# JacobYoung115/VisualSLAM

Hardware: AMD Instinct MI355X
Metric: frames/sec @1080p (Harris + DoG keypoint detection) (higher is better)
Workload: dtype u8

## Files before the change

visualslam_amd/csrc/kernels_aux.hip.h:

```cpp
#pragma once
#include <hip/hip_runtime.h>

#include "kernels_generic.hip.h"
#include "kernels_localize.hip.h"

namespace vslam {

__global__ __launch_bounds__(256) void k_resize_linear2x_slide(const uint8_t* __restrict__ src, size_t sstep, size_t sframe,
                                                                uint8_t* __restrict__ dst, size_t dframe, int dpitch,
                                                                int rows, int cols, int seg) {
    const int k = blockIdx.x * 256 + threadIdx.x;
    if (4 * k >= cols) return;
    const bool whole = 4 * k + 3 < cols;
    const int m0 = blockIdx.y * seg, m1 = min(m0 + seg, rows);
    const uint8_t* s = src + blockIdx.z * sframe;
    uint8_t* d = dst + blockIdx.z * dframe + 8 * k;
    const int xl = max(4 * k - 1, 0), xr = min(4 * k + 4, cols - 1);
    auto hrow = [&](int m, uint32_t (&X)[4], uint32_t (&Y)[4]) {
        const uint8_t* r = s + (size_t)min(max(m, 0), rows - 1) * sstep;
        uint32_t w;
        if (whole)
            __builtin_memcpy(&w, r + 4 * k, 4);
        else
            w = (uint32_t)r[4 * k] | ((uint32_t)r[min(4 * k + 1, cols - 1)] << 8) | ((uint32_t)r[min(4 * k + 2, cols - 1)] << 16) |
// ... 12 lines not shown
            Y[i] = pk_lshr_u16(A[i] + (A[i] << 1), 2);
        }
    };
    auto emit = [&](int dy, const uint32_t (&U)[4], const uint32_t (&V)[4]) {
        uint32_t v[4];
#pragma unroll
        for (int i = 0; i < 4; ++i) v[i] = pk_lshr_u16(U[i] + V[i] + 0x00020002u, 2);
        *reinterpret_cast<uint2*>(d + (size_t)dy * dpitch) = make_uint2(v[0] | (v[1] << 8), v[2] | (v[3] << 8));
    };
    uint32_t Xp[4], Yp[4], Xc[4], Yc[4];
    hrow(m0 - 1, Xp, Yp);
    hrow(m0, Xc, Yc);
    for (int m = m0; m < m1; ++m) {
        uint32_t Xn[4], Yn[4];
        hrow(m + 1, Xn, Yn);
        emit(2 * m, Xp, Yc);
        emit(2 * m + 1, Yc, Xn);
#pragma unroll
        for (int i = 0; i < 4; ++i) Xp[i] = Xc[i], Xc[i] = Xn[i], Yc[i] = Yn[i];
    }
}

__global__ __launch_bounds__(256) void k_resize_nearest_half_v4(const uint8_t* __restrict__ src, size_t sframe, int spitch,
                                                                 uint8_t* __restrict__ dst, size_t dframe, int dpitch,
                                                                 int rows, int drows, int dcols) {
    const int k = blockIdx.x * 256 + threadIdx.x;
    const int y = blockIdx.y;
    if (4 * k >= dcols) return;
    const int sy = min(2 * y, rows - 1);
    const uint2 w = *reinterpret_cast<const uint2*>(src + blockIdx.z * sframe + (size_t)sy * spitch + 8 * k);
    *reinterpret_cast<uint32_t*>(dst + blockIdx.z * dframe + (size_t)y * dpitch + 4 * k) =
        even_bytes(w.x, w.y);
}

constexpr int EXT_SPAN = 768;
constexpr int EXT_PITCH = EXT_SPAN + 16;

template <bool LOC>
__global__ __launch_bounds__(256) void k_extrema_w3(const uint8_t* __restrict__ pyr, size_t pframe, ExtGeom g, int o,
                                                     unsigned long long* __restrict__ bits,
                                                     unsigned long long* __restrict__ lflags, size_t bframe, int li0, int li_step) {
    constexpr int NROW = LOC ? 13 : 10;
    __shared__ __attribute__((aligned(16))) uint8_t srow[NROW * EXT_PITCH + 16];
    __shared__ uint2 queue[LOC ? 768 : 1];
    __shared__ uint8_t qkeep[LOC ? 768 : 1];
    const int li = li0 + (int)blockIdx.y * li_step, f = blockIdx.z;
    const int rows = g.rows[o], cols = g.cols[o], pitch = g.pitch[o];
    const uint32_t P = (uint32_t)rows * (uint32_t)pitch;
    const uint8_t* dog = pyr + f * pframe + g.oct_off[o] + (size_t)VSLAM_NUM_LEVELS * P;
    const int ya = max(3 * li - 1, 0), yb = 3 * li;
    const int yc = min(3 * li + 1, rows - 1);
    const int c0 = blockIdx.x * EXT_SPAN - 16;
    const int wave = __builtin_amdgcn_readfirstlane(threadIdx.x >> 6), lane = threadIdx.x & 63;
    const int cpiece = c0 + 16 * lane;
    const bool piece_ok = lane < EXT_PITCH / 16 && cpiece >= 0 && cpiece < cols;
#pragma unroll
    for (int i = 0; i < (NROW + 3) / 4; ++i) {
        const int rl = wave + 4 * i;
        if (rl < NROW) {
            const int lev = rl < 10 ? (rl >> 1) : rl - 9, y = rl < 10 ? ((rl & 1) ? yb : ya) : yc;
            const uint8_t* rowp = dog + (ptrdiff_t)(int)((uint32_t)lev * P + (uint32_t)y * (uint32_t)pitch + (uint32_t)c0);
            if (piece_ok)
                *reinterpret_cast<uint4*>(srow + rl * EXT_PITCH + 16 * lane) =
                    *reinterpret_cast<const uint4*>(rowp + (uint32_t)(16 * lane));
        }
    }
    if (blockIdx.x == 0 && threadIdx.x < 10)
        srow[threadIdx.x * EXT_PITCH + 15] = dog[(threadIdx.x >> 1) * P + (uint32_t)((threadIdx.x & 1) ? yb : ya) * (uint32_t)pitch];
    __syncthreads();
    const int lc = g.lat_cols[o], wpr = g.wpr[o], lr = g.lat_rows[o];
    const int lj = blockIdx.x * 256 + threadIdx.x;
    bool cand[3] = {false, false, false}, listed[3] = {false, false, false};
    unsigned long long wcand[3], wlist[3];
    const unsigned long long owns = __builtin_amdgcn_ballot_w64(lj < lc);
    const int xa = 3 * (int)threadIdx.x - 1 + 16;
    uint32_t self[5];
    uint32_t up[5], left[5];
    {
        const uint32_t s = xa & 3;
        const uint32_t sel = 0x0c000c00u | s | ((s + 1) << 16);
        uint32_t mn[5], mx[5];
#pragma unroll
        for (int l = 0; l < 5; ++l) {
            uint32_t off = (uint32_t)(xa & ~3) + (uint32_t)(2 * l * EXT_PITCH);
            if (l) asm volatile("" : "+v"(off));
            const uint32_t* q0 = reinterpret_cast<const uint32_t*>(srow + off);
            const uint32_t* q1 = q0 + EXT_PITCH / 4;
            const uint32_t v0 = __builtin_amdgcn_perm(q0[1], q0[0], sel), v1 = __builtin_amdgcn_perm(q1[1], q1[0], sel);
            const uint32_t lo = pk_min_u16(v0, v1), hi = pk_max_u16(v0, v1);
            mn[l] = min(lo & 0xffffu, lo >> 16);
            mx[l] = max(hi & 0xffffu, hi >> 16);
            self[l] = v1 >> 16;
            if (LOC) up[l] = v0 >> 16, left[l] = v1 & 0xffffu;
        }
#pragma unroll
        for (int L = 1; L <= 3; ++L) {
            const uint32_t lo = min(mn[L - 1], min(mn[L], mn[L + 1])), hi = max(mx[L - 1], max(mx[L], mx[L + 1]));
            wcand[L - 1] = (__builtin_amdgcn_ballot_w64(self[L] == lo) | __builtin_amdgcn_ballot_w64(self[L] == hi)) & owns;
            if (LOC) cand[L - 1] = lj < lc && (self[L] == lo || self[L] == hi);
            else wlist[L - 1] = wcand[L - 1] & __builtin_amdgcn_ballot_w64((int)self[L] >= g.min_contrast);
        }
    }
    if (LOC) {
        uint2* wq = queue + wave * 192;
        uint8_t* wk = qkeep + wave * 192;
        const int xj = xa + 1;
        const int xr = xj + ((3 * lj + 1 < cols) ? 1 : 0);
        unsigned int nw = 0;
        bool queued[3];
#pragma unroll
        for (int L = 1; L <= 3; ++L) {
            bool nz = false;
            uint32_t dpack = 0;
            if (cand[L - 1]) {
                const uint8_t* r1 = srow + (2 * L + 1) * EXT_PITCH;
                const uint8_t* r2 = srow + (9 + L) * EXT_PITCH;
                const int d_x = (int)left[L] - (int)r1[xr];
                const int d_y = (int)up[L] - (int)r2[xj];
                const int d_s = (int)self[L - 1] - (int)self[L + 1];
                nz = d_x != 0 && d_y != 0 && d_s != 0;
                listed[L - 1] = !nz && self[L] >= 8u;
                dpack = (uint32_t)(d_x + 256) | ((uint32_t)(d_y + 256) << 10) | ((uint32_t)(d_s + 256) << 20);
            }
            const unsigned long long m = __builtin_amdgcn_ballot_w64(nz);
            if (nz) {
                const unsigned int slot = nw + __builtin_amdgcn_mbcnt_hi((uint32_t)(m >> 32), __builtin_amdgcn_mbcnt_lo((uint32_t)m, 0u));
                wq[slot] = make_uint2(dpack, self[L] | ((uint32_t)((L - 1) * 64 + lane) << 8));
            }
            queued[L - 1] = nz;
            nw += (unsigned int)__builtin_popcountll(m);
        }
        if (nw) {
            __builtin_amdgcn_fence(__ATOMIC_RELEASE, "wavefront");
            __builtin_amdgcn_wave_barrier();
            __builtin_amdgcn_fence(__ATOMIC_ACQUIRE, "wavefront");
            for (unsigned int q = lane; q < nw; q += 64) {
                const uint2 e = wq[q];
                int nv;
                wk[e.y >> 8] = feature_point_localization((int)(e.x & 1023u) - 256, (int)((e.x >> 10) & 1023u) - 256,
                                                          (int)(e.x >> 20) - 256, (int)(e.y & 255u), nv, g.loc_lut);
            }
            __builtin_amdgcn_fence(__ATOMIC_RELEASE, "wavefront");
            __builtin_amdgcn_wave_barrier();
            __builtin_amdgcn_fence(__ATOMIC_ACQUIRE, "wavefront");
#pragma unroll
            for (int L = 0; L < 3; ++L)
                if (queued[L]) listed[L] = wk[L * 64 + lane] != 0;
        }
    }
    const int word = blockIdx.x * 4 + wave;
    if (word < wpr) {
        const size_t w0 = f * bframe + g.bits_off[o] + (size_t)li * wpr + word;
#pragma unroll
        for (int L = 0; L < 3; ++L) {
            const unsigned long long wc = wcand[L], wl = LOC ? __builtin_amdgcn_ballot_w64(listed[L]) : wlist[L];
            if (lane == 0) {
                const size_t w = w0 + (size_t)L * lr * wpr;
                if (bits) bits[w] = wc;
                lflags[w] = wl;
            }
        }
    }
}


template <bool FMA>
__device__ __forceinline__ float mad_f32(float a, float b, float c) {
    if constexpr (FMA) return __builtin_fmaf(a, b, c);
    else return a * b + c;
}

template <bool FMA = false>
__device__ __forceinline__ float fast_atan2_deg(float y, float x) {
    const float scale = (float)(180.0 / 3.14159265358979323846);
    const float p1 = 0.9997878412794807f * scale, p3 = -0.3258083974640975f * scale;
    const float p5 = 0.1555786518463281f * scale, p7 = -0.04432655554792128f * scale;
    const float eps = (float)2.2204460492503131e-16;
    const float ax = fabsf(x), ay = fabsf(y);
    float a;
    if (ax >= ay) {
        const float c = ay / (ax + eps), c2 = c * c;
        a = mad_f32<FMA>(mad_f32<FMA>(mad_f32<FMA>(p7, c2, p5), c2, p3), c2, p1) * c;
    } else {
        const float c = ax / (ay + eps), c2 = c * c;
        a = 90.f - mad_f32<FMA>(mad_f32<FMA>(mad_f32<FMA>(p7, c2, p5), c2, p3), c2, p1) * c;
    }
    if (x < 0) a = 180.f - a;
    if (y < 0) a = 360.f - a;
    return a;
}

template <int BINS>
__device__ __forceinline__ int hist_bin(float deg) {
    const float reductionCoeff = (float)BINS / 360.0f;
    const int index = (int)(deg * reductionCoeff);
    return min(max(index, 0), BINS - 1);
}

__device__ __forceinline__ float gradient_magnitude(float gx, float gy) {
    const float xx = gx * gx, yy = gy * gy;
    return sqrt_rn_small_nr(xx + yy);
}

template <class Geom>
__device__ __forceinline__ const uint8_t* level_plane(const uint8_t* __restrict__ pyr, int f, size_t pframe, const Geom& g, int o, int level) {
    return pyr + f * pframe + g.oct_off[o] + (size_t)level * g.rows[o] * g.pitch[o];
}

template <bool FMA>
__global__ __launch_bounds__(256) void k_level_gradients(const uint8_t* __restrict__ g, int gpitch, int rows, int cols,
                                                          float* __restrict__ gx, float* __restrict__ gy,
                                                          float* __restrict__ mag, float* __restrict__ orient) {
    const int c = blockIdx.x * 256 + threadIdx.x;
    const int r = blockIdx.y;
// ... 12 lines not shown
```

visualslam_amd/csrc/kernels_pyramid.hip.h:

```cpp
#pragma once
#include <hip/hip_runtime.h>

#include "kernels_generic.hip.h"

namespace vslam {

template <int TW_, int TH_, int N0, int N1, int N2, int N3, int N4, int N5>
struct PyrCfg {
    static constexpr int TW = TW_, TH = TH_;
    static constexpr int n(int l) { return l == 0 ? N0 : l == 1 ? N1 : l == 2 ? N2 : l == 3 ? N3 : l == 4 ? N4 : N5; }
    static constexpr int cmax(int a, int b) { return a > b ? a : b; }
    static constexpr int NMAX = cmax(cmax(cmax(N0, N1), cmax(N2, N3)), cmax(N4, N5));
    static constexpr int R = (NMAX / 2 + 15) & ~15;
    static constexpr int RQ = (TH + 2 * R) / 4;
    static constexpr int RW = TW + 2 * R;
    static constexpr int RWP = RW + 4;
    static constexpr int r(int l) { return n(l) / 2; }
    static constexpr int delta(int l) { return (R - r(l)) & 3; }
    static constexpr int A(int l) { return (R - r(l)) & ~3; }
    static constexpr int ncg(int l) { return (TW + 2 * r(l) + delta(l) + 3) / 4; }
    static constexpr int m1(int l) { return ((delta(l) + 3 + n(l) - 1) >> 2) + 1; }
    static constexpr int pmax(int l) { return (7 + delta(l) + 2 * r(l)) / 2; }
    static constexpr int nb(int l) { return pmax(l) / 4 + 1; }
    static constexpr int hpp_l(int l) { return cmax(2 * ncg(l), TW / 2 - 4 + 4 * nb(l)); }
    static constexpr int HPP =
        (cmax(cmax(cmax(hpp_l(0), hpp_l(1)), cmax(hpp_l(2), hpp_l(3))), cmax(hpp_l(4), hpp_l(5))) + 15) & ~15;
    static constexpr int T4M = ((3 + NMAX - 1) >> 2) + 1;
    static constexpr int TPM = NMAX + 1;
    static constexpr int LDS_BYTES = (RQ * RWP + TH * HPP) * 4;
    static constexpr int NT = (TH / 4) * (TW / 8);
    static constexpr int NW = NT / 64;
    static_assert(TW % 16 == 0 && TH % 8 == 0 && NT % 256 == 0 && NT <= 1024,
                  "a multiple of four waves, one per SIMD: 384-thread workgroups (384 x 32 tiles) ran 16 % slower, their six waves sit 2-2-1-1");
    static_assert((N0 & 1) && (N1 & 1) && (N2 & 1) && (N3 & 1) && (N4 & 1) && (N5 & 1), "odd kernels");
};

template <class CFG>
struct PyrTaps {
    uint32_t t4[6][4][CFG::T4M];
    uint32_t tp[6][CFG::TPM];
};

template <class CFG, int L>
__device__ __forceinline__ void pyr_level(const PyrTaps<CFG>* __restrict__ taps, const uint32_t* __restrict__ rp,
                                          uint32_t* __restrict__ hp, uint8_t* __restrict__ out, size_t P, int cols,
                                          int pitch, int rows, int tile_x0, int tile_y0, uint32_t (&prev_e)[4][2],
                                          uint32_t (&prev_o)[4][2], uint8_t* __restrict__ next_base, int nrows,
                                          int ncols, int npitch, const uint32_t (&row_off)[4]) {
    constexpr int n = CFG::n(L), dl = CFG::delta(L), A = CFG::A(L);
    constexpr int NCG = CFG::ncg(L), M = CFG::m1(L), NB = CFG::nb(L);
    constexpr int RWP = CFG::RWP, HPP = CFG::HPP, TH = CFG::TH;
    const int tid = threadIdx.x;
    uint32_t z1;
    asm volatile("s_mov_b32 %0, 0" : "=s"(z1));
    const uint32_t* __restrict__ t4 = &taps->t4[L][0][0] + z1;
    const uint4* __restrict__ rp4 = reinterpret_cast<const uint4*>(rp);

    constexpr int NT = CFG::NT;
    constexpr int N1 = NCG * (TH / 4), FULL1 = N1 / NT * NT;
    for (int k = 0; k < (N1 + NT - 1) / NT; ++k) {
        int it = tid + NT * k;
        if (k == N1 / NT) {
            it = FULL1 + (tid + NT - 64 * (L % CFG::NW)) % NT;
            if (it >= N1) break;
        }
        const int cg = it % NCG, rq = it / NCG;
        uint32_t acc[4][4];
#pragma unroll
        for (int j = 0; j < 4; ++j)
#pragma unroll
            for (int c = 0; c < 4; ++c) acc[j][c] = 0;
        const uint4* col = rp4 + (rq + A / 4) * (RWP / 4) + cg + A / 4;
#pragma unroll
        for (int m = 0; m < M; ++m) {
            const uint4 v = col[m * (RWP / 4)];
#pragma unroll
            for (int j = 0; j < 4; ++j) {
                const int s = dl + j, o = s & 3, mm = m - (s >> 2);
                if (mm >= 0 && mm <= ((o + n - 1) >> 2)) {
                    const uint32_t t = t4[o * CFG::T4M + mm];
                    acc[j][0] = udot4(v.x, t, acc[j][0]);
                    acc[j][1] = udot4(v.y, t, acc[j][1]);
                    acc[j][2] = udot4(v.z, t, acc[j][2]);
                    acc[j][3] = udot4(v.w, t, acc[j][3]);
                }
            }
        }
#pragma unroll
        for (int j = 0; j < 4; ++j) {
            uint2 w;
            w.x = __builtin_amdgcn_perm(acc[j][1], acc[j][0], 0x05040100);
            w.y = __builtin_amdgcn_perm(acc[j][3], acc[j][2], 0x05040100);
            *reinterpret_cast<uint2*>(hp + (4 * rq + j) * HPP + 2 * cg) = w;
        }
    }
    __syncthreads();

    uint32_t z2;
    asm volatile("s_mov_b32 %0, 0" : "=s"(z2));
    const uint32_t* __restrict__ tp = &taps->tp[L][0] + z2;
    const int xg = tid % (CFG::TW / 8), rg = tid / (CFG::TW / 8);
    uint32_t acc[4][8];
#pragma unroll
    for (int jr = 0; jr < 4; ++jr)
#pragma unroll
        for (int j = 0; j < 8; ++j) acc[jr][j] = 32768u;
#pragma unroll
    for (int b = 0; b < NB; ++b) {
        uint32_t zb = 0;
        if (CFG::TPM > 40 && (b & 1) == 0) asm volatile("s_mov_b32 %0, 0" : "=s"(zb));
        const uint32_t* __restrict__ tpb = CFG::TPM > 40 ? tp + zb : tp;
#pragma unroll
        for (int jr = 0; jr < 4; ++jr) {
            const uint4 v = *reinterpret_cast<const uint4*>(hp + (4 * rg + jr) * HPP + 4 * xg + 4 * b);
            asm volatile("" ::"v"(v.x), "v"(v.y), "v"(v.z), "v"(v.w));
            const uint32_t vv[4] = {v.x, v.y, v.z, v.w};
#pragma unroll
            for (int pp = 0; pp < 4; ++pp) {
#pragma unroll
                for (int j = 0; j < 8; ++j) {
                    const int e = 2 * (4 * b + pp) - j - dl + 1;
                    if (e >= 0 && e <= n) acc[jr][j] = udot2(vv[pp], tpb[e], acc[jr][j]);
                }
            }
        }
    }
    __syncthreads();

    const int x = tile_x0 + 8 * xg;
#pragma unroll
    for (int jr = 0; jr < 4; ++jr) {
        const int y = tile_y0 + 4 * rg + jr;
        uint32_t g[2], d[2];
#pragma unroll
        for (int hw = 0; hw < 2; ++hw)
            level_pack4(acc[jr][4 * hw], acc[jr][4 * hw + 1], acc[jr][4 * hw + 2], acc[jr][4 * hw + 3], L, g[hw], d[hw], prev_e[jr][hw],
                        prev_o[jr][hw]);
        if (y < rows && x < cols) {
            const uint32_t off = row_off[jr];
            uint8_t* gp = out + (size_t)L * P;
            *reinterpret_cast<uint2*>(gp + off) = make_uint2(g[0], g[1]);
            if (L > 0) {
                uint8_t* dp = out + (size_t)(VSLAM_NUM_LEVELS + L - 1) * P;
                *reinterpret_cast<uint2*>(dp + off) = make_uint2(d[0], d[1]);
            }
            if (L == 3 && next_base && (jr & 1) == 0 && (y >> 1) < nrows && (x >> 1) < ncols)
                *reinterpret_cast<uint32_t*>(next_base + ((uint32_t)(y >> 1) * (uint32_t)npitch + (uint32_t)(x >> 1))) = even_bytes(g[0], g[1]);
        }
    }
}

template <class CFG>
__global__ __launch_bounds__(CFG::NT) void k_pyr_octave(const uint8_t* __restrict__ base, size_t bframe,
                                                     uint8_t* __restrict__ oct_out, size_t pframe, int rows, int cols,
                                                     int pitch, const PyrTaps<CFG>* __restrict__ taps,
                                                     uint8_t* __restrict__ next_base, size_t nframe, int nrows, int ncols,
                                                     int npitch) {
    extern __shared__ __attribute__((aligned(16))) uint32_t smem[];
    uint32_t* rp = smem;
    uint32_t* hp = smem + CFG::RQ * CFG::RWP;
    constexpr int R = CFG::R, RW = CFG::RW, RWP = CFG::RWP, RQ = CFG::RQ;
    const int tid = threadIdx.x;
    unsigned int bid = blockIdx.x + gridDim.x * (blockIdx.y + gridDim.y * blockIdx.z);
    const unsigned int per_xcd = (gridDim.x * gridDim.y * gridDim.z) >> 3;
    if (bid < (per_xcd << 3)) bid = (bid & 7u) * per_xcd + (bid >> 3);
    const unsigned int tiles_per_frame = gridDim.x * gridDim.y;
    const unsigned int fz = bid / tiles_per_frame, rem = bid - fz * tiles_per_frame;
    const unsigned int by = rem / gridDim.x, bx = rem - by * gridDim.x;
    const int tile_x0 = bx * CFG::TW, tile_y0 = by * CFG::TH;
    const uint8_t* src = base + fz * bframe;
    uint8_t* out = oct_out + fz * pframe;
    const size_t P = (size_t)rows * pitch;

    const bool interior = tile_x0 - R >= 0 && tile_x0 + CFG::TW + R <= cols && tile_y0 - R >= 0 &&
                          tile_y0 + CFG::TH + R <= rows;
// ... 10 lines not shown
                *reinterpret_cast<uint4*>(rp + yq * RWP + 16 * xs + 4 * q) = transpose4x4_u8(aw[0][q], aw[1][q], aw[2][q], aw[3][q]);
        }
    } else if (cols >= 4 && R < cols && tile_x0 + CFG::TW + R - 1 <= 2 * (cols - 1) && R < rows && tile_y0 + CFG::TH + R - 1 <= 2 * (rows - 1)) {
        auto f1 = [](int x, int n) { return x < 0 ? -x : (x >= n ? 2 * (n - 1) - x : x); };
#pragma unroll 2
        for (int it = tid; it < RQ * (RW / 4); it += CFG::NT) {
            const int yq = it / (RW / 4), xq = it - yq * (RW / 4);
            const int gy = tile_y0 - R + 4 * yq, gx = tile_x0 - R + 4 * xq;
            const int p0 = f1(gx, cols), p1 = f1(gx + 1, cols), p2 = f1(gx + 2, cols), p3 = f1(gx + 3, cols);
            const int b0 = min(min(min(p0, p1), min(p2, p3)), cols - 4);
            const uint32_t sel = (uint32_t)(p0 - b0) | ((uint32_t)(p1 - b0) << 8) | ((uint32_t)(p2 - b0) << 16) | ((uint32_t)(p3 - b0) << 24);
            uint32_t a[4];
#pragma unroll
            for (int k = 0; k < 4; ++k) {
                uint32_t v;
                __builtin_memcpy(&v, src + (size_t)f1(gy + k, rows) * pitch + b0, 4);
                a[k] = __builtin_amdgcn_perm(0u, v, sel);
            }
            *reinterpret_cast<uint4*>(rp + yq * RWP + 4 * xq) = transpose4x4_u8(a[0], a[1], a[2], a[3]);
        }
    } else {
        for (int it = tid; it < RQ * (RW / 4); it += CFG::NT) {
            const int yq = it / (RW / 4), xq = it - yq * (RW / 4);
            const int gy = tile_y0 - R + 4 * yq, gx = tile_x0 - R + 4 * xq;
            uint32_t a[4];
#pragma unroll
            for (int k = 0; k < 4; ++k) {
                const uint8_t* row = src + (size_t)reflect101(gy + k, rows) * pitch;
                a[k] = (uint32_t)row[reflect101(gx, cols)] | ((uint32_t)row[reflect101(gx + 1, cols)] << 8) |
                       ((uint32_t)row[reflect101(gx + 2, cols)] << 16) | ((uint32_t)row[reflect101(gx + 3, cols)] << 24);
            }
            *reinterpret_cast<uint4*>(rp + yq * RWP + 4 * xq) = transpose4x4_u8(a[0], a[1], a[2], a[3]);
        }
    }
    __syncthreads();

    uint8_t* nb = next_base ? next_base + fz * nframe : nullptr;
    uint32_t prev_e[4][2], prev_o[4][2];
    uint32_t row_off[4];
    {
        const int xg = tid % (CFG::TW / 8), rg = tid / (CFG::TW / 8);
#pragma unroll
        for (int jr = 0; jr < 4; ++jr)
            row_off[jr] = (uint32_t)(tile_y0 + 4 * rg + jr) * (uint32_t)pitch + (uint32_t)(tile_x0 + 8 * xg);
    }
    pyr_level<CFG, 0>(taps, rp, hp, out, P, cols, pitch, rows, tile_x0, tile_y0, prev_e, prev_o, nb, nrows, ncols, npitch, row_off);
    pyr_level<CFG, 1>(taps, rp, hp, out, P, cols, pitch, rows, tile_x0, tile_y0, prev_e, prev_o, nb, nrows, ncols, npitch, row_off);
    pyr_level<CFG, 2>(taps, rp, hp, out, P, cols, pitch, rows, tile_x0, tile_y0, prev_e, prev_o, nb, nrows, ncols, npitch, row_off);
    pyr_level<CFG, 3>(taps, rp, hp, out, P, cols, pitch, rows, tile_x0, tile_y0, prev_e, prev_o, nb, nrows, ncols, npitch, row_off);
    pyr_level<CFG, 4>(taps, rp, hp, out, P, cols, pitch, rows, tile_x0, tile_y0, prev_e, prev_o, nb, nrows, ncols, npitch, row_off);
    pyr_level<CFG, 5>(taps, rp, hp, out, P, cols, pitch, rows, tile_x0, tile_y0, prev_e, prev_o, nb, nrows, ncols, npitch, row_off);
}

static inline uint32_t pack_taps_u8x4(const uint16_t* t, int n, int m, int o) {
    uint32_t w = 0;
    for (int b = 0; b < 4; ++b) {
        const int k = 4 * m + b - o;
        if (k >= 0 && k < n) w |= (uint32_t)(t[k] & 0xff) << (8 * b);
    }
    return w;
}
static inline uint32_t pack_taps_u16x2(const uint16_t* t, int n, int e) {
    const uint32_t lo = (e >= 1 && e - 1 < n) ? t[e - 1] : 0, hi = (e >= 0 && e < n) ? t[e] : 0;
    return lo | (hi << 16);
}

template <class CFG>
static void pyr_pack_taps(const uint16_t* const t[6], PyrTaps<CFG>& out) {
    for (int l = 0; l < 6; ++l) {
        for (int o = 0; o < 4; ++o)
            for (int m = 0; m < CFG::T4M; ++m) out.t4[l][o][m] = pack_taps_u8x4(t[l], CFG::n(l), m, o);
        for (int e = 0; e < CFG::TPM; ++e) out.tp[l][e] = pack_taps_u16x2(t[l], CFG::n(l), e);
    }
}

using PyrCfgOct0 = PyrCfg<128, 64, 9, 13, 15, 19, 23, 29>;
using PyrCfgOct1 = PyrCfg<128, 64, 19, 23, 29, 37, 45, 57>;
using PyrCfgOct0W = PyrCfg<256, 32, 9, 13, 15, 19, 23, 29>;
using PyrCfgOct1W = PyrCfg<256, 32, 19, 23, 29, 37, 45, 57>;

}
```

visualslam_amd/csrc/vslam_hip.hip:

```cpp
#include <hip/hip_runtime.h>

#include <algorithm>
#include <cstdio>
#include <cstdlib>
#include <cstring>
#include <deque>
#include <map>
#include <string>
#include <set>
#include <memory>
#include <vector>

#include "../../include/vslam.h"
#include "kernels_generic.hip.h"
#include "kernels_pyramid.hip.h"
#include "kernels_strip.hip.h"
#include "kernels_hdiff.hip.h"
#include "kernels_aux.hip.h"
#include "kernels_harris_strip.hip.h"
#include "kernels_orient.hip.h"
#include "kernels_orient_batch.hip.h"
#include "kernels_orient_pk.hip.h"
#include "kernels_compact.hip.h"
#include "kernels_sift.hip.h"
// ... 109 lines not shown
    return fail(ctx, VSLAM_ERR_UNSUPPORTED, std::string(what) + ": its tap tables are not on the device yet and cannot be put there during a stream capture - " \
                                                                "run one warm-up call with the same parameters and the same matrix-path setting first")

enum TableKind { kTableBlur, kTableStrip, kTableTile, kTableMx, kTableOrient };

template <class T, class Fill>
static int get_table(vslam_ctx* c, TableKind kind, double v, int i, const char* what, size_t bytes, Fill fill, const T** out) {
    uint64_t vb;
    std::memcpy(&vb, &v, 8);
    const auto key = std::make_tuple((int)kind, vb, i);
    auto it = c->tables.find(key);
    if (it == c->tables.end()) {
        NO_TABLE_IN_CAPTURE(c, what);
        std::vector<char> host(bytes);
        TRY(fill(static_cast<void*>(host.data())));
        void* d = nullptr;
        HIPCHK(c, hipMalloc(&d, bytes));
        HIPCHK(c, hipMemcpy(d, host.data(), bytes, hipMemcpyHostToDevice));
        it = c->tables.emplace(key, d).first;
    }
    *out = static_cast<const T*>(it->second);
    return VSLAM_OK;
}

static inline void tap_pointers(const std::vector<uint16_t> taps[6], const uint16_t* tp[6]) {
    for (int l = 0; l < 6; ++l) tp[l] = taps[l].data();
}

static int get_taps(vslam_ctx* c, int n, double sigma, const uint16_t** out, int* n_eff) {
    std::vector<uint16_t> h;
    if (!gauss_taps_q8_trimmed(n, sigma, h)) return fail(c, VSLAM_ERR_INVALID, "invalid Gaussian kernel size");
    *n_eff = (int)h.size();
    return get_table(c, kTableBlur, sigma, n, "Gaussian blur", sizeof(uint16_t) * h.size(), [&](void* host) -> int {
        std::memcpy(host, h.data(), sizeof(uint16_t) * h.size());
        return VSLAM_OK;
    }, out);
}

static inline dim3 grid_rows(int cols, int rows, int frames = 1) { return dim3((cols + 255) / 256, rows, frames); }


namespace {
enum class OctPath { Tile0, Tile1, Strip, Generic };

struct OctPlan {
    OctPath path = OctPath::Generic;
    int ks[6] = {};
    double sg[6] = {};
    int ke[6] = {};
    std::vector<uint16_t> taps[6];
    int nmax = 0;
    int sh = 0;
    int hdiff = 0;
    int mx = 0;
};
}

static bool taps_fit_u8(const OctPlan& pl) {
    for (int l = 0; l < 6; ++l)
        for (uint16_t v : pl.taps[l])
            if (v > 255) return false;
    return true;
}

template <class CFG>
static bool matches_cfg(const int ks[6]) {
    for (int l = 0; l < 6; ++l)
        if (ks[l] != CFG::n(l)) return false;
    return true;
}

static OctPlan plan_octave(double sigma0, int o, int rows, int cols) {
    OctPlan pl;
    int& nmax = pl.nmax;
    for (int l = 0; l < 6; ++l) {
        pl.sg[l] = sigma_at(sigma0, o, l);
        pl.ks[l] = gauss_ksize_u8(pl.sg[l]);
        if (!gauss_taps_q8_trimmed(pl.ks[l], pl.sg[l], pl.taps[l])) return pl;
        pl.ke[l] = (int)pl.taps[l].size();
        nmax = std::max(nmax, pl.ke[l]);
    }
    if (!taps_fit_u8(pl)) return pl;
    if (matches_cfg<PyrCfgOct0>(pl.ke)) {
        pl.path = OctPath::Tile0;
    } else if (matches_cfg<PyrCfgOct1>(pl.ke)) {
        pl.path = OctPath::Tile1;
    } else if (nmax <= STRIP_MAXN) {
        pl.sh = strip_plan_sh(rows, cols, nmax);
        if (pl.sh) pl.path = OctPath::Strip;
        if (pl.path == OctPath::Strip && hdiff_fits(cols) && hdiff_stage_fits(cols))
            pl.hdiff = hd_octave_matches<2>(pl.taps) ? 2 : hd_octave_matches<3>(pl.taps) ? 3 : 0;
    }
    if (pl.path != OctPath::Generic) pl.mx = mx_config_for(pl.ke);
    return pl;
}

static std::vector<OctPlan> plan_octaves(double sigma0, const vslam_batch_layout& L) {
    std::vector<OctPlan> plans;
    for (int o = 0; o < L.n_octaves; ++o) plans.push_back(plan_octave(sigma0, o, L.rows[o], L.cols[o]));
    return plans;
}

template <int SH, int RI>
static int launch_h_strip(vslam_ctx* c, const uint16_t* h, size_t hframe, const OctIO& io, const StripLaunch& sl, const StripTaps* taps) {
    TRY(raise_dyn_lds(c, reinterpret_cast<const void*>(&k_gauss_h_strip<SH, RI>)));
    LAUNCH_ON(c, "k_gauss_h_strip", c->launch_tag, c->stream, sl.h_lds, (k_gauss_h_strip<SH, RI>), dim3(1, sl.h_grid_y, io.nf), dim3(256), h,
              hframe, io.oct, io.pframe, io.rows, io.cols, io.pitch, sl.pw, taps, io.next_base, io.nframe, io.nrows, io.ncols, io.npitch);
    return VSLAM_OK;
}

template <int O>
static int launch_h_diff(vslam_ctx* c, const uint16_t* h, size_t hframe, const OctIO& io, const StripLaunch& sl) {
    TRY(raise_dyn_lds(c, reinterpret_cast<const void*>(&k_gauss_h_diff<O>)));
    TimedScope ts(c, "k_gauss_h_strip", c->launch_tag);
    LAUNCH_ON(c, "k_gauss_h_diff", c->launch_tag, c->stream, sl.h_lds, k_gauss_h_diff<O>, dim3(1, sl.h_grid_y, io.nf), dim3(256), h,
              hframe, io.oct, io.pframe, io.rows, io.cols, io.pitch, sl.npairs, sl.pw, io.next_base, io.nframe, io.nrows, io.ncols, io.npitch);
    return VSLAM_OK;
}

static int enqueue_strip_octave(vslam_ctx* c, double sigma0, int o, const OctPlan& pl, const OctIO& io, uint16_t* h) {
    const StripTaps* taps;
    TRY(get_table(c, kTableStrip, sigma0, o, "strip kernels", sizeof(StripTaps), [&](void* host) -> int {
        const uint16_t* tp[6];
        tap_pointers(pl.taps, tp);
        if (!strip_pack_taps(tp, pl.ke, *static_cast<StripTaps*>(host))) return fail(c, VSLAM_ERR_UNSUPPORTED, "strip kernels: taps out of range");
        return VSLAM_OK;
    }, &taps));
    const int rows = io.rows, cols = io.cols, nf = io.nf;
    static const bool hdiff_off = [] {
        const char* e = VSLAM_DIAG_ENV("VSLAM_HDIFF");
        return e && e[0] == '0';
    }();
    const int hd = hdiff_off ? 0 : pl.hdiff;
    const StripLaunch sl = hd == 2   ? strip_launch(rows, cols, nf, pl.sh, true, pl.nmax, HdGeom<2>::HL, HdGeom<2>::rmax)
                           : hd == 3 ? strip_launch(rows, cols, nf, pl.sh, true, pl.nmax, HdGeom<3>::HL, HdGeom<3>::rmax)
                                     : strip_launch(rows, cols, nf, pl.sh, false, pl.nmax);
    const StripVGeom vg = strip_v_geom(rows, pl.nmax);
    const size_t P = (size_t)rows * io.pitch;
    TRY(raise_dyn_lds(c, reinterpret_cast<const void*>(&k_gauss_v_strip)));
// ... 102 lines not shown
    size_t site_frame = 0, site_off[VSLAM_MAX_OCTAVES] = {};
    int site_pitch[VSLAM_MAX_OCTAVES] = {};
    uint8_t* colmap = nullptr;
    size_t col_frame = 0, col_off[VSLAM_MAX_OCTAVES] = {};
};

static inline int site_pitch_of(int lat_cols) { return (lat_cols + 63) & ~63; }
static size_t col_octave_bytes(const vslam_batch_layout& L, int o) { return align_up((size_t)5 * mx_seams(L.cols[o]) * L.rows[o] * 2, 16); }

static size_t dog_h_elems(const vslam_batch_layout& L, const std::vector<OctPlan>& plans) {
    size_t m = 0;
    for (int o = 0; o < L.n_octaves; ++o) {
        const size_t P = (size_t)L.rows[o] * L.pitch[o];
        if (plans[o].path == OctPath::Strip) m = std::max(m, 6 * P);
        if (plans[o].path == OctPath::Generic) m = std::max(m, P);
    }
    return m;
}

static void dog_scratch_plan(WsPlan& ws, const vslam_batch_layout& L, const std::vector<OctPlan>& plans, int nf, DogScratch& s, bool sitemap = false) {
    if (sitemap) {
        size_t off = 0;
        for (int o = 0; o < L.n_octaves; ++o) {
            s.site_off[o] = off;
            s.site_pitch[o] = site_pitch_of(L.lat_cols[o]);
            off += (size_t)L.lat_rows[o] * s.site_pitch[o];
        }
        s.site_frame = off;
        ws.add(s.sitemap, (size_t)nf * off);
        size_t coff = 0;
        for (int o = 0; o < L.n_octaves; ++o) {
            s.col_off[o] = coff;
            coff += col_octave_bytes(L, o);
        }
        s.col_frame = coff;
        ws.add(s.colmap, (size_t)nf * coff + 16);
    }
    size_t sum_p = 0;
    for (int o = 0; o < L.n_octaves; ++o) {
        s.base_off[o] = sum_p;
        sum_p += (size_t)L.rows[o] * L.pitch[o];
    }
    s.bases_frame = sum_p;
    ws.add(s.bases, (size_t)nf * sum_p);
    ws.add(s.h, (size_t)nf * dog_h_elems(L, plans) + 128);
    ws.add(s.lflags, (size_t)nf * L.bits_frame_words);
    ws.add(s.cws, compaction_ws_elems(L.bits_frame_words, nf));
    ws.add(s.pbegin, nf);
}


template <class CFG>
static int enqueue_pyr_octave(vslam_ctx* c, double sigma0, int o, const OctPlan& pl, const OctIO& io) {
    const PyrTaps<CFG>* taps;
    TRY(get_table(c, kTableTile, sigma0, o, "octave kernel", sizeof(PyrTaps<CFG>), [&](void* host) -> int {
        const uint16_t* tp[6];
        tap_pointers(pl.taps, tp);
        pyr_pack_taps<CFG>(tp, *static_cast<PyrTaps<CFG>*>(host));
        return VSLAM_OK;
    }, &taps));
    TRY(raise_dyn_lds(c, reinterpret_cast<const void*>(&k_pyr_octave<CFG>)));
    const dim3 grid((io.cols + CFG::TW - 1) / CFG::TW, (io.rows + CFG::TH - 1) / CFG::TH, io.nf);
    LAUNCH_ON(c, "k_pyr_octave", o, c->stream, CFG::LDS_BYTES, k_pyr_octave<CFG>, grid, dim3(CFG::NT), io.base, io.bframe, io.oct, io.pframe, io.rows,
              io.cols, io.pitch, taps, io.next_base, io.nframe, io.nrows, io.ncols, io.npitch);
    return VSLAM_OK;
}

static int enqueue_pyr_octave_mx(vslam_ctx* c, double sigma0, int o, const OctPlan& pl, const OctIO& io, const MxScan* scan, int up2_step = 0) {
    const void* table;
    TRY(get_table(c, kTableMx, sigma0, o, "matrix-core octave kernel", mx_taps_bytes(pl.mx), [&](void* host) -> int {
        const uint16_t* tp[6];
        tap_pointers(pl.taps, tp);
        if (!mx_pack(pl.mx, tp, host)) return fail(c, VSLAM_ERR_UNSUPPORTED, "matrix-core octave kernel: a tap exceeds 127");
        HIPCHK(c, mx_prepare(pl.mx));
        return VSLAM_OK;
    }, &table));
    hipError_t e;
    {
        TimedScope ts(c, "k_pyr_octave_mx", o);
        e = mx_launch(pl.mx, c->stream, table, io, scan, up2_step);
    }
    HIPCHK(c, e);
    return VSLAM_OK;
}

static DenseGeom dense_geom(const vslam_batch_layout& L, int o, int min_contrast, int nf) {
    DenseGeom g;
    g.rows = L.rows[o], g.cols = L.cols[o], g.pitch = L.pitch[o];
    g.wpr = (g.cols + 63) / 64;
    g.min_contrast = min_contrast;
    g.P = (unsigned int)((size_t)g.rows * g.pitch);
    g.dog_off = (unsigned int)(L.octave_offset[o] + (size_t)VSLAM_NUM_LEVELS * g.P);
    const long waves_per_rowseg = 4L * (((g.cols + 3) / 4 + 255) / 256) * nf;
    const long segs_wanted = std::max<long>(1, 8192 / waves_per_rowseg);
    g.seg = (int)std::min<long>(XD_SEG_MAX, std::max<long>(4, (g.rows + segs_wanted - 1) / segs_wanted));
    return g;
}

namespace {
struct DogOut {
    uint8_t* pyr;
    size_t pframe;
    unsigned long long* bits = nullptr;
    bool do_extrema = false;
    vslam_point* points = nullptr;
    unsigned int* counts = nullptr;
};

static inline hipStream_t lane_stream(const vslam_ctx* c, Lane l) { return l == Lane::Main ? c->stream : c->aux[(int)l - 1]; }

static BatchPlanIn batch_plan_input(const vslam_ctx* c, const vslam_params& p, const vslam_batch_layout& L, const std::vector<OctPlan>& plans, size_t fstep) {
    BatchPlanIn in;
    in.n_octaves = L.n_octaves;
// ... 69 lines not shown
                TimedScope ts(c, "k_extrema_w3", o, es);
                if (n_straddle > 0)
                    hipLaunchKernelGGL(k_extrema_w3<false>, dim3((L.lat_words[o] + 3) / 4, n_straddle, nf), dim3(256), 0, es, pyr, pframe, g, o, bits, s.lflags,
                                       L.bits_frame_words, sr, sr);
                if (on_side) HIPCHK(c, hipEventRecord(c->ev_pack, es));
            } else if (p.extrema_window == 3) {
                const dim3 eg((L.lat_words[o] + 3) / 4, L.lat_rows[o], nf);
                if (p.localize)
                    LAUNCH_ON(c, "k_extrema_w3", o, es, 0, k_extrema_w3<true>, eg, dim3(256), pyr, pframe, g, o, bits, s.lflags, L.bits_frame_words, 0, 1);
                else
                    LAUNCH_ON(c, "k_extrema_w3", o, es, 0, k_extrema_w3<false>, eg, dim3(256), pyr, pframe, g, o, bits, s.lflags, L.bits_frame_words, 0, 1);
            } else
                hipLaunchKernelGGL(k_extrema, dim3((L.lat_cols[o] + 255) / 256, L.lat_rows[o], nf * 3), dim3(256), 0, es, pyr,
                                   pframe, g, o, bits, s.lflags, L.bits_frame_words);
            HIPCHK(c, hipGetLastError());
        }
        if (out.do_extrema && out.points && out.counts) {
            StreamSwap sw(c, es);
            const size_t entries = (size_t)3 * L.lat_rows[o] * L.lat_words[o];
            if (p.extrema_dense) {
                DenseDogEntries ent{s.lflags + L.bits_offset[o], L.bits_frame_words, pyr, pframe, dense_geom(L, o, p.min_contrast, nf), o, out.points};
                TRY(enqueue_compaction(c, ent, entries, nf, s.cws, p.dog_cap, out.counts, o > 0 ? 1 : 0));
            } else {
                DogEntries ent{s.lflags, L.bits_frame_words, pyr, pframe, g, o, o + 1, out.points};
                TRY(enqueue_compaction(c, ent, entries, nf, s.cws, p.dog_cap, out.counts, o > 0 ? 1 : 0));
            }
        }
        return VSLAM_OK;
    }

    int octave(vslam_ctx* c, int o) {
        const int nf_a = plan.nf_a;
        const int rows = L.rows[o], cols = L.cols[o], pitch = L.pitch[o];
        const size_t P = (size_t)rows * pitch;
        const OctPlan& pl = plans[o];
        const bool has_next = o + 1 < L.n_octaves;
        const bool fuse_next = has_next && pl.path != OctPath::Generic;
        OctIO io{s.bases + s.base_off[o], s.bases_frame, out.pyr + L.octave_offset[o], out.pframe, rows, cols, pitch, nf,
                 fuse_next ? s.bases + s.base_off[o + 1] : nullptr, s.bases_frame, has_next ? L.rows[o + 1] : 0, has_next ? L.cols[o + 1] : 0,
                 has_next ? L.pitch[o + 1] : 0};
        const bool up2 = o == 0 && plan.up2_fused;
        if (up2) io.base = frames, io.bframe = fframe;
        const int shape = pyr_tile_wide(rows, cols) ? 1 : 0;
        const bool fused = plan.fused[o];
        auto tiled = [&](int f_lo, int n) -> int {
            const OctIO part = io.frames(f_lo, n);
            if (c->mx && pl.mx) {
                MxScan sc = scan[o];
                if (fused) sc.sitemap += (size_t)f_lo * s.site_frame, sc.colmap += (size_t)f_lo * s.col_frame;
                return enqueue_pyr_octave_mx(c, p.sigma0, o, pl, part, fused ? &sc : nullptr, up2 ? (int)fstep : 0);
            }
            if (pl.path == OctPath::Tile0)
                return shape == 1 ? enqueue_pyr_octave<PyrCfgOct0W>(c, p.sigma0, o, pl, part) : enqueue_pyr_octave<PyrCfgOct0>(c, p.sigma0, o, pl, part);
            return shape == 1 ? enqueue_pyr_octave<PyrCfgOct1W>(c, p.sigma0, o, pl, part) : enqueue_pyr_octave<PyrCfgOct1>(c, p.sigma0, o, pl, part);
        };
        const bool is_tiled = pl.path == OctPath::Tile0 || pl.path == OctPath::Tile1 || (c->mx && pl.mx != 0);
        if (o == 0 && nf_a < nf && !is_tiled) HIPCHK(c, hipStreamWaitEvent(c->stream, c->ev_up2, 0));
        if (is_tiled && o == 0 && nf_a < nf) {
            TRY(tiled(0, nf_a));
            HIPCHK(c, hipStreamWaitEvent(c->stream, c->ev_up2, 0));
            TRY(tiled(nf_a, nf - nf_a));
        } else if (is_tiled)
            TRY(tiled(0, nf));
        else if (pl.path == OctPath::Strip)
            TRY(enqueue_strip_octave(c, p.sigma0, o, pl, io, s.h));
        else {
            for (int l = 0; l < VSLAM_NUM_LEVELS; ++l)
                TRY(enqueue_blur(c, io.base, (size_t)pitch, s.bases_frame, io.oct + (size_t)l * P, (size_t)pitch, out.pframe, s.h, rows,
                                 cols, nf, pl.ks[l], pl.sg[l]));
            LAUNCH(c, "k_dog5", k_dog5, dim3((unsigned)((P + 255) / 256), 1, nf), dim3(256), io.oct,
                   io.oct + (size_t)VSLAM_NUM_LEVELS * P, P, out.pframe);
        }
        if (has_next && !fuse_next)
            LAUNCH(c, "k_resize_nearest_half_v4", k_resize_nearest_half_v4, dim3((L.cols[o + 1] / 4 + 256) / 256, L.rows[o + 1], nf),
                   dim3(256), io.oct + (size_t)3 * P, out.pframe, pitch, s.bases + s.base_off[o + 1], s.bases_frame, L.pitch[o + 1], rows,
                   L.rows[o + 1], L.cols[o + 1]);
        if (plan.ev_oct) HIPCHK(c, hipEventRecord(c->ev_oct[o], c->stream));
        if (o == 0) TRY(sched_mark_phase(c));
        return VSLAM_OK;
    }
};

struct HarrisChunk {
    const uint8_t* frames;
    size_t fframe;
    int rows, cols, nf;
    float k, *resp;
    uint8_t* mask;
    float* nms2;
    unsigned long long* hflags;
    vslam_kp* kps;
    unsigned int cap, *counts, *cws;
};
}


struct OrientPlan;
struct OrientScratch;
static int enqueue_dog(vslam_ctx* c, DogChunk& d, const HarrisChunk* hc = nullptr, const OrientPlan* opl = nullptr, OrientScratch* os = nullptr);

static int enqueue_harris(vslam_ctx* c, const uint8_t* frames, size_t fframe, int rows, int cols, int nf, float k,
                          float* resp, uint8_t* mask, float* nms2, unsigned long long* hflags, vslam_kp* kps,
                          unsigned int cap, unsigned int* counts, unsigned int* chunk_ws) {
    const size_t N = (size_t)rows * cols;
    if (N >= ((size_t)1 << 31)) return fail(c, VSLAM_ERR_UNSUPPORTED, "Harris: images of 2^31 pixels or more are not supported (32-bit row offsets)");
    const HarrisLaunch g = harris_launch(rows, cols, nf, fframe);
// ... 1163 lines not shown
```

Measured before the change: 15190.

## Compile octave-1 blur taps as constants and streamline extrema staging

Adds a compile-time tap table for octave 1 when the runtime taps match the generated defaults. The tiled pyramid kernel then uses immediate constants instead of loading taps from a device table. The extrema kernel now shares min/max reductions across adjacent levels with packed ops, computes the ownership mask arithmetically instead of by ballot, and handles the first column's left border through the byte-permute selector, which drops a separate scalar load. It also simplifies the bitmask stores. The constant-tap path only runs when the taps match, and it is skipped entirely when the matrix-core path is selected, so its effect depends on configuration.

```diff
diff --git a/visualslam_amd/csrc/kernels_aux.hip.h b/visualslam_amd/csrc/kernels_aux.hip.h
--- a/visualslam_amd/csrc/kernels_aux.hip.h
+++ b/visualslam_amd/csrc/kernels_aux.hip.h
@@ -88,34 +88,40 @@
     const int yc = min(3 * li + 1, rows - 1);
     const int c0 = blockIdx.x * EXT_SPAN - 16;
     const int wave = __builtin_amdgcn_readfirstlane(threadIdx.x >> 6), lane = threadIdx.x & 63;
-    const int cpiece = c0 + 16 * lane;
-    const bool piece_ok = lane < EXT_PITCH / 16 && cpiece >= 0 && cpiece < cols;
+    uint32_t piece = 16u * (uint32_t)lane;
+    asm volatile("" : "+v"(piece));
+    const bool piece_ok = lane < EXT_PITCH / 16 && (uint32_t)c0 + piece < (uint32_t)cols;
+    uint8_t* const sdst = srow + wave * EXT_PITCH + piece;
 #pragma unroll
     for (int i = 0; i < (NROW + 3) / 4; ++i) {
         const int rl = wave + 4 * i;
         if (rl < NROW) {
             const int lev = rl < 10 ? (rl >> 1) : rl - 9, y = rl < 10 ? ((rl & 1) ? yb : ya) : yc;
-            const uint8_t* rowp = dog + (ptrdiff_t)(int)((uint32_t)lev * P + (uint32_t)y * (uint32_t)pitch + (uint32_t)c0);
-            if (piece_ok)
-                *reinterpret_cast<uint4*>(srow + rl * EXT_PITCH + 16 * lane) =
-                    *reinterpret_cast<const uint4*>(rowp + (uint32_t)(16 * lane));
-        }
-    }
-    if (blockIdx.x == 0 && threadIdx.x < 10)
-        srow[threadIdx.x * EXT_PITCH + 15] = dog[(threadIdx.x >> 1) * P + (uint32_t)((threadIdx.x & 1) ? yb : ya) * (uint32_t)pitch];
+            uint64_t rowp = reinterpret_cast<uint64_t>(dog + (ptrdiff_t)(int)((uint32_t)lev * P + (uint32_t)y * (uint32_t)pitch + (uint32_t)c0));
+            asm volatile("" : "+s"(rowp));
+            typedef uint32_t piece_t __attribute__((ext_vector_type(4)));
+            typedef const piece_t __attribute__((address_space(1))) * global_piece;
+            if (piece_ok) *reinterpret_cast<piece_t*>(sdst + 4 * i * EXT_PITCH) = *reinterpret_cast<global_piece>(rowp + piece);
+        }
+    }
     __syncthreads();
     const int lc = g.lat_cols[o], wpr = g.wpr[o], lr = g.lat_rows[o];
     const int lj = blockIdx.x * 256 + threadIdx.x;
+    const int word = blockIdx.x * 4 + wave;
     bool cand[3] = {false, false, false}, listed[3] = {false, false, false};
     unsigned long long wcand[3], wlist[3];
-    const unsigned long long owns = __builtin_amdgcn_ballot_w64(lj < lc);
+    const int nown = lc - 64 * word;
+    const unsigned long long owns = nown >= 64 ? ~0ull : nown > 0 ? (1ull << nown) - 1ull : 0ull;
     const int xa = 3 * (int)threadIdx.x - 1 + 16;
     uint32_t self[5];
     uint32_t up[5], left[5];
     {
         const uint32_t s = xa & 3;
-        const uint32_t sel = 0x0c000c00u | s | ((s + 1) << 16);
-        uint32_t mn[5], mx[5];
+        int xfirst = blockIdx.x == 0 ? 16 : 0;
+        asm volatile("" : "+s"(xfirst));
+        const uint32_t sa = s + (xa < xfirst ? 1u : 0u);
+        const uint32_t sel = 0x0c010c00u + sa + (s << 16);
+        uint32_t plo[5], phi[5];
 #pragma unroll
         for (int l = 0; l < 5; ++l) {
             uint32_t off = (uint32_t)(xa & ~3) + (uint32_t)(2 * l * EXT_PITCH);
@@ -123,15 +129,17 @@
             const uint32_t* q0 = reinterpret_cast<const uint32_t*>(srow + off);
             const uint32_t* q1 = q0 + EXT_PITCH / 4;
             const uint32_t v0 = __builtin_amdgcn_perm(q0[1], q0[0], sel), v1 = __builtin_amdgcn_perm(q1[1], q1[0], sel);
-            const uint32_t lo = pk_min_u16(v0, v1), hi = pk_max_u16(v0, v1);
-            mn[l] = min(lo & 0xffffu, lo >> 16);
-            mx[l] = max(hi & 0xffffu, hi >> 16);
+            plo[l] = pk_min_u16(v0, v1), phi[l] = pk_max_u16(v0, v1);
             self[l] = v1 >> 16;
             if (LOC) up[l] = v0 >> 16, left[l] = v1 & 0xffffu;
         }
+        const uint32_t lo12 = pk_min_u16(plo[1], plo[2]), hi12 = pk_max_u16(phi[1], phi[2]);
+        const uint32_t lo34 = pk_min_u16(plo[3], plo[4]), hi34 = pk_max_u16(phi[3], phi[4]);
+        const uint32_t wlo[3] = {pk_min_u16(plo[0], lo12), pk_min_u16(lo12, plo[3]), pk_min_u16(plo[2], lo34)};
+        const uint32_t whi[3] = {pk_max_u16(phi[0], hi12), pk_max_u16(hi12, phi[3]), pk_max_u16(phi[2], hi34)};
 #pragma unroll
         for (int L = 1; L <= 3; ++L) {
-            const uint32_t lo = min(mn[L - 1], min(mn[L], mn[L + 1])), hi = max(mx[L - 1], max(mx[L], mx[L + 1]));
+            const uint32_t lo = min(wlo[L - 1] & 0xffffu, wlo[L - 1] >> 16), hi = max(whi[L - 1] & 0xffffu, whi[L - 1] >> 16);
             wcand[L - 1] = (__builtin_amdgcn_ballot_w64(self[L] == lo) | __builtin_amdgcn_ballot_w64(self[L] == hi)) & owns;
             if (LOC) cand[L - 1] = lj < lc && (self[L] == lo || self[L] == hi);
             else wlist[L - 1] = wcand[L - 1] & __builtin_amdgcn_ballot_w64((int)self[L] >= g.min_contrast);
@@ -184,18 +192,20 @@
                 if (queued[L]) listed[L] = wk[L * 64 + lane] != 0;
         }
     }
-    const int word = blockIdx.x * 4 + wave;
-    if (word < wpr) {
-        const size_t w0 = f * bframe + g.bits_off[o] + (size_t)li * wpr + word;
-#pragma unroll
-        for (int L = 0; L < 3; ++L) {
-            const unsigned long long wc = wcand[L], wl = LOC ? __builtin_amdgcn_ballot_w64(listed[L]) : wlist[L];
-            if (lane == 0) {
-                const size_t w = w0 + (size_t)L * lr * wpr;
-                if (bits) bits[w] = wc;
-                lflags[w] = wl;
-            }
-        }
+    if (LOC) {
+#pragma unroll
+        for (int L = 0; L < 3; ++L) wlist[L] = __builtin_amdgcn_ballot_w64(listed[L]);
+    }
+    if (word < wpr && lane == 0) {
+        const uint32_t lw = (uint32_t)lr * (uint32_t)wpr, e0 = (uint32_t)li * (uint32_t)wpr + (uint32_t)word;
+        unsigned long long* const lf = lflags + f * bframe + g.bits_off[o] + e0;
+        if (bits) {
+            unsigned long long* const bw = bits + f * bframe + g.bits_off[o] + e0;
+#pragma unroll
+            for (int L = 0; L < 3; ++L) bw[(size_t)L * lw] = wcand[L];
+        }
+#pragma unroll
+        for (int L = 0; L < 3; ++L) lf[(size_t)L * lw] = wlist[L];
     }
 }
 
diff --git a/visualslam_amd/csrc/kernels_pyramid.hip.h b/visualslam_amd/csrc/kernels_pyramid.hip.h
--- a/visualslam_amd/csrc/kernels_pyramid.hip.h
+++ b/visualslam_amd/csrc/kernels_pyramid.hip.h
@@ -1,6 +1,7 @@
 #pragma once
 #include <hip/hip_runtime.h>
 
+#include "diff_taps.gen.h"
 #include "kernels_generic.hip.h"
 
 namespace vslam {
@@ -8,6 +9,7 @@
 template <int TW_, int TH_, int N0, int N1, int N2, int N3, int N4, int N5>
 struct PyrCfg {
     static constexpr int TW = TW_, TH = TH_;
+    static constexpr int DO = 0;
     static constexpr int n(int l) { return l == 0 ? N0 : l == 1 ? N1 : l == 2 ? N2 : l == 3 ? N3 : l == 4 ? N4 : N5; }
     static constexpr int cmax(int a, int b) { return a > b ? a : b; }
     static constexpr int NMAX = cmax(cmax(cmax(N0, N1), cmax(N2, N3)), cmax(N4, N5));
@@ -41,6 +43,43 @@
     uint32_t tp[6][CFG::TPM];
 };
 
+static inline constexpr uint32_t pack_taps_u8x4(const uint16_t* t, int n, int m, int o) {
+    uint32_t w = 0;
+    for (int b = 0; b < 4; ++b) {
+        const int k = 4 * m + b - o;
+        if (k >= 0 && k < n) w |= (uint32_t)(t[k] & 0xff) << (8 * b);
+    }
+    return w;
+}
+static inline constexpr uint32_t pack_taps_u16x2(const uint16_t* t, int n, int e) {
+    const uint32_t lo = (e >= 1 && e - 1 < n) ? t[e - 1] : 0, hi = (e >= 0 && e < n) ? t[e] : 0;
+    return lo | (hi << 16);
+}
+
+template <class BASE, int O>
+struct PyrCfgConst : BASE {
+    static constexpr int DO = O;
+};
+
+template <class CFG, int L>
+struct PyrLevelTaps {
+    uint32_t t4[4][CFG::T4M];
+    uint32_t tp[CFG::TPM];
+    constexpr PyrLevelTaps() : t4{}, tp{} {
+        using LV = dtaps::Lvl<CFG::DO, L>;
+        static_assert(LV::n == CFG::n(L), "the compiled-in taps have the configuration's widths");
+        for (int o = 0; o < 4; ++o)
+            for (int m = 0; m < CFG::T4M; ++m) t4[o][m] = pack_taps_u8x4(LV::w, LV::n, m, o);
+        for (int e = 0; e < CFG::TPM; ++e) tp[e] = pack_taps_u16x2(LV::w, LV::n, e);
+    }
+};
+
+template <class CFG, int L>
+__device__ __forceinline__ const PyrLevelTaps<CFG, L>& level_taps() {
+    static constexpr PyrLevelTaps<CFG, L> k{};
+    return k;
+}
+
 template <class CFG, int L>
 __device__ __forceinline__ void pyr_level(const PyrTaps<CFG>* __restrict__ taps, const uint32_t* __restrict__ rp,
                                           uint32_t* __restrict__ hp, uint8_t* __restrict__ out, size_t P, int cols,
@@ -51,9 +90,10 @@
     constexpr int NCG = CFG::ncg(L), M = CFG::m1(L), NB = CFG::nb(L);
     constexpr int RWP = CFG::RWP, HPP = CFG::HPP, TH = CFG::TH;
     const int tid = threadIdx.x;
-    uint32_t z1;
-    asm volatile("s_mov_b32 %0, 0" : "=s"(z1));
-    const uint32_t* __restrict__ t4 = &taps->t4[L][0][0] + z1;
+    constexpr bool CT = CFG::DO != 0;
+    uint32_t z1 = 0;
+    if constexpr (!CT) asm volatile("s_mov_b32 %0, 0" : "=s"(z1));
+    const uint32_t* __restrict__ t4 = CT ? nullptr : &taps->t4[L][0][0] + z1;
     const uint4* __restrict__ rp4 = reinterpret_cast<const uint4*>(rp);
 
     constexpr int NT = CFG::NT;
@@ -78,7 +118,9 @@
             for (int j = 0; j < 4; ++j) {
                 const int s = dl + j, o = s & 3, mm = m - (s >> 2);
                 if (mm >= 0 && mm <= ((o + n - 1) >> 2)) {
-                    const uint32_t t = t4[o * CFG::T4M + mm];
+                    uint32_t t;
+                    if constexpr (CT) t = level_taps<CFG, L>().t4[o][mm];
+                    else t = t4[o * CFG::T4M + mm];
                     acc[j][0] = udot4(v.x, t, acc[j][0]);
                     acc[j][1] = udot4(v.y, t, acc[j][1]);
                     acc[j][2] = udot4(v.z, t, acc[j][2]);
@@ -96,9 +138,9 @@
     }
     __syncthreads();
 
-    uint32_t z2;
-    asm volatile("s_mov_b32 %0, 0" : "=s"(z2));
-    const uint32_t* __restrict__ tp = &taps->tp[L][0] + z2;
+    uint32_t z2 = 0;
+    if constexpr (!CT) asm volatile("s_mov_b32 %0, 0" : "=s"(z2));
+    const uint32_t* __restrict__ tp = CT ? nullptr : &taps->tp[L][0] + z2;
     const int xg = tid % (CFG::TW / 8), rg = tid / (CFG::TW / 8);
     uint32_t acc[4][8];
 #pragma unroll
@@ -108,7 +150,7 @@
 #pragma unroll
     for (int b = 0; b < NB; ++b) {
         uint32_t zb = 0;
-        if (CFG::TPM > 40 && (b & 1) == 0) asm volatile("s_mov_b32 %0, 0" : "=s"(zb));
+        if (!CT && CFG::TPM > 40 && (b & 1) == 0) asm volatile("s_mov_b32 %0, 0" : "=s"(zb));
         const uint32_t* __restrict__ tpb = CFG::TPM > 40 ? tp + zb : tp;
 #pragma unroll
         for (int jr = 0; jr < 4; ++jr) {
@@ -120,7 +162,10 @@
 #pragma unroll
                 for (int j = 0; j < 8; ++j) {
                     const int e = 2 * (4 * b + pp) - j - dl + 1;
-                    if (e >= 0 && e <= n) acc[jr][j] = udot2(vv[pp], tpb[e], acc[jr][j]);
+                    if (e >= 0 && e <= n) {
+                        if constexpr (CT) acc[jr][j] = udot2(vv[pp], level_taps<CFG, L>().tp[e], acc[jr][j]);
+                        else acc[jr][j] = udot2(vv[pp], tpb[e], acc[jr][j]);
+                    }
                 }
             }
         }
@@ -237,19 +282,6 @@
     pyr_level<CFG, 5>(taps, rp, hp, out, P, cols, pitch, rows, tile_x0, tile_y0, prev_e, prev_o, nb, nrows, ncols, npitch, row_off);
 }
 
-static inline uint32_t pack_taps_u8x4(const uint16_t* t, int n, int m, int o) {
-    uint32_t w = 0;
-    for (int b = 0; b < 4; ++b) {
-        const int k = 4 * m + b - o;
-        if (k >= 0 && k < n) w |= (uint32_t)(t[k] & 0xff) << (8 * b);
-    }
-    return w;
-}
-static inline uint32_t pack_taps_u16x2(const uint16_t* t, int n, int e) {
-    const uint32_t lo = (e >= 1 && e - 1 < n) ? t[e - 1] : 0, hi = (e >= 0 && e < n) ? t[e] : 0;
-    return lo | (hi << 16);
-}
-
 template <class CFG>
 static void pyr_pack_taps(const uint16_t* const t[6], PyrTaps<CFG>& out) {
     for (int l = 0; l < 6; ++l) {
@@ -263,5 +295,7 @@
 using PyrCfgOct1 = PyrCfg<128, 64, 19, 23, 29, 37, 45, 57>;
 using PyrCfgOct0W = PyrCfg<256, 32, 9, 13, 15, 19, 23, 29>;
 using PyrCfgOct1W = PyrCfg<256, 32, 19, 23, 29, 37, 45, 57>;
-
-}
+using PyrCfgOct1C = PyrCfgConst<PyrCfgOct1, 1>;
+using PyrCfgOct1WC = PyrCfgConst<PyrCfgOct1W, 1>;
+
+}
diff --git a/visualslam_amd/csrc/vslam_hip.hip b/visualslam_amd/csrc/vslam_hip.hip
--- a/visualslam_amd/csrc/vslam_hip.hip
+++ b/visualslam_amd/csrc/vslam_hip.hip
@@ -185,6 +185,7 @@
     int nmax = 0;
     int sh = 0;
     int hdiff = 0;
+    int ctaps = 0;
     int mx = 0;
 };
 }
@@ -218,6 +219,7 @@
         pl.path = OctPath::Tile0;
     } else if (matches_cfg<PyrCfgOct1>(pl.ke)) {
         pl.path = OctPath::Tile1;
+        pl.ctaps = hd_octave_matches<1>(pl.taps) ? 1 : 0;
     } else if (nmax <= STRIP_MAXN) {
         pl.sh = strip_plan_sh(rows, cols, nmax);
         if (pl.sh) pl.path = OctPath::Strip;
@@ -426,13 +428,14 @@
 
 template <class CFG>
 static int enqueue_pyr_octave(vslam_ctx* c, double sigma0, int o, const OctPlan& pl, const OctIO& io) {
-    const PyrTaps<CFG>* taps;
-    TRY(get_table(c, kTableTile, sigma0, o, "octave kernel", sizeof(PyrTaps<CFG>), [&](void* host) -> int {
-        const uint16_t* tp[6];
-        tap_pointers(pl.taps, tp);
-        pyr_pack_taps<CFG>(tp, *static_cast<PyrTaps<CFG>*>(host));
-        return VSLAM_OK;
-    }, &taps));
+    const PyrTaps<CFG>* taps = nullptr;
+    if constexpr (CFG::DO == 0)
+        TRY(get_table(c, kTableTile, sigma0, o, "octave kernel", sizeof(PyrTaps<CFG>), [&](void* host) -> int {
+            const uint16_t* tp[6];
+            tap_pointers(pl.taps, tp);
+            pyr_pack_taps<CFG>(tp, *static_cast<PyrTaps<CFG>*>(host));
+            return VSLAM_OK;
+        }, &taps));
     TRY(raise_dyn_lds(c, reinterpret_cast<const void*>(&k_pyr_octave<CFG>)));
     const dim3 grid((io.cols + CFG::TW - 1) / CFG::TW, (io.rows + CFG::TH - 1) / CFG::TH, io.nf);
     LAUNCH_ON(c, "k_pyr_octave", o, c->stream, CFG::LDS_BYTES, k_pyr_octave<CFG>, grid, dim3(CFG::NT), io.base, io.bframe, io.oct, io.pframe, io.rows,
@@ -608,6 +611,8 @@
             }
             if (pl.path == OctPath::Tile0)
                 return shape == 1 ? enqueue_pyr_octave<PyrCfgOct0W>(c, p.sigma0, o, pl, part) : enqueue_pyr_octave<PyrCfgOct0>(c, p.sigma0, o, pl, part);
+            if (pl.ctaps == 1)
+                return shape == 1 ? enqueue_pyr_octave<PyrCfgOct1WC>(c, p.sigma0, o, pl, part) : enqueue_pyr_octave<PyrCfgOct1C>(c, p.sigma0, o, pl, part);
             return shape == 1 ? enqueue_pyr_octave<PyrCfgOct1W>(c, p.sigma0, o, pl, part) : enqueue_pyr_octave<PyrCfgOct1>(c, p.sigma0, o, pl, part);
         };
         const bool is_tiled = pl.path == OctPath::Tile0 || pl.path == OctPath::Tile1 || (c->mx && pl.mx != 0);
```

Measured after the change: 15400 (median of 6 runs). 1.01x the previous value.
